# facebookresearch/foundpose

Measured on AMD Instinct MI355X. Metric: detections/sec (ViT+kNN match) on 518^2 crops vs 10k-template bank, higher is better.
Workload: dtype bf16; 1 GPU; tie_order=torch

## Files before the change

### foundpose_amd/_lib.py

```python

import ctypes as C
import os

import torch

_HERE = os.path.dirname(os.path.abspath(__file__))
LIB_PATH = os.environ.get("FOUNDPOSE_AMD_LIB") or os.path.join(_HERE, "lib", "libfoundpose_amd.so")

FP_F32, FP_BF16, FP_FP8, FP_F16X3, FP_F16F8, FP_F16 = 0, 1, 2, 3, 4, 5
GEMM_SPLIT_F16F8 = 1 << 20
GEMM_F16 = 1 << 21
SPLIT_SCALE_ACT, SPLIT_SCALE_QKV, SPLIT_SCALE_HID = 16.0, 16.0, 4.0
ABI_VERSION = 20

vp, i32, i64, f32, f64, u64 = C.c_void_p, C.c_int, C.c_int64, C.c_float, C.c_double, C.c_uint64


class VitBlock(C.Structure):
    _fields_ = [(n, vp) for n in (
        "ln1_w", "ln1_b", "ln2_w", "ln2_b", "ls1", "ls2",
        "qkv_w", "proj_w", "fc1_w", "fc2_w",
        "qkv_b", "proj_b", "fc1_b", "fc2_b", "qkv_s", "proj_s", "fc1_s", "fc2_s")] + [("act_scale", f32 * 4), ("qkv_colsum", vp), ("fc1_colsum", vp)]


# ... 23 lines not shown
    "fp_cosine_topk_prefiltered": [vp, vp, vp, i32, i32, vp, vp, vp, i32, i32, i32, i32, vp, vp, vp, i32, vp],
    "fp_cyclic_buddies": [vp, vp, vp, vp, i32, i32, vp, vp, vp, i32, vp, vp, vp, vp, i32, i32, i32, i32,
                          vp, vp, vp, vp, vp, vp, vp, vp, i32, vp],
    "fp_pack_records": [vp, vp, vp, vp, vp, vp, vp, vp, vp, i32, i32, i32, vp, vp],
    "fp_pnp_ransac": [vp, vp, vp, vp, i32, i32, i32, i32, f64, f64, i32, i32, u64, vp, vp, vp, vp, vp, vp, vp],
    "fp_pnp_ransac_keyed": [vp, vp, vp, vp, vp, i32, i32, i32, i32, f64, f64, i32, i32, u64, vp, vp, vp, vp, vp, vp, vp],
    "fp_kabsch_ransac": [vp, vp, vp, vp, vp, vp, vp, vp, vp, i32, i32, i32, vp, i32, i32, i32, i32, f64, i32, i32, u64, vp, vp, vp, vp, vp, vp, vp, vp],
    "fp_pose_verify_depth": [vp, vp, vp, vp, vp, vp, vp, vp, vp, vp, vp, i32, vp, i32, i32, i32, i32, i32, i32, i32, vp, vp, vp, vp],
    "fp_pose_verify_mask": [vp, vp, vp, vp, vp, vp, vp, vp, vp, i32, vp, vp, i32, i32, i32, i32, i32, i32, vp, vp, vp, vp],
    "fp_sample_bilinear": [vp, i64, i64, i64, i64, i32, i32, i32, i32, i32, vp, vp, i32, vp, vp],
    "fp_pca_project": [vp, i32, i32, vp, i32, vp, vp, vp],
    "fp_vit_forward": [C.POINTER(VitModel), C.POINTER(VitWorkspace), vp, i32, i32, i32, i32, vp],
    "fp_vit_sample_features": [C.POINTER(VitModel), C.POINTER(VitWorkspace), i32, i32, i32, i32, i32, i32, vp, vp, i32, vp, vp],
    "fp_query_select": [vp, i32, i32, i32, vp, vp, vp, i32, vp, i32, i32, vp, vp, vp, vp, vp, vp, vp, vp, vp],
    "fp_vit_forward_prefix": [C.POINTER(VitModel), C.POINTER(VitWorkspace), vp, i32, i32, i32, i32, vp],
    "fp_vit_block_selected": [C.POINTER(VitModel), C.POINTER(VitWorkspace), i32, i32, i32, i32, vp, vp, i32, i32, vp],
    "fp_vit_sample_features_selected": [C.POINTER(VitModel), C.POINTER(VitWorkspace), i32, i32, i32, i32, i32, i32, vp, vp, i32, vp, vp, vp],
    "fp_vit_features": [C.POINTER(VitModel), C.POINTER(VitWorkspace), i32, i32, i32, vp, vp, vp],
    "fp_patchify": [vp, i32, i32, i32, i32, vp, i32, i32, vp],
    "fp_layernorm": [vp, i32, vp, vp, f32, vp, i32, i32, i32, i32, i32, i32, i32, vp],
    "fp_gemm_bf16": [vp, i32, vp, i32, i32, i32, i32, i32, vp, vp, vp, i32, i32, vp],
    "fp_gemm_bf16_ln": [vp, i32, vp, i32, i32, i32, i32, i32, vp, vp, i32, i32, vp, vp, vp, i32, vp, vp],
    "fp_gemm_resid_tile_rows": [i32, i32, i32],
    "fp_ln_finalize": [vp, i32, i32, i32, i32, f32, vp, vp],
    "fp_gemm_fp8": [vp, i32, vp, i32, i32, i32, i32, i32, vp, vp, vp, i32, i32, f32, vp],
    "fp_quantize_fp8": [vp, i32, i64, f32, vp, vp],
    "fp_gemm_split": [vp, i32, vp, i32, i32, i32, i32, i32, vp, vp, vp, i32, i32, f32, f32, vp],
    "fp_attention_split": [vp, i32, vp, i32, i32, i32, i32, i32, f32, f32, i32, vp],
    "fp_layernorm_scaled": [vp, i32, vp, vp, f32, vp, i32, i32, f32, i32, i32, vp],
    "fp_gemm_f32": [vp, i32, vp, i32, i32, i32, i32, vp, vp, vp, i32, i32, vp],
    "fp_attention": [vp, i32, vp, i32, i32, i32, i32, i32, i32, vp],
    "fp_convert_f32_to_bf16": [vp, vp, i64, vp],
    "fp_warp_crops": [vp, i32, i32, i32, i32, i32, vp, vp, i32, i32, i32, i32, vp, vp, vp],
    "fp_warp_depth": [vp, i32, i32, vp, vp, i32, i32, i32, i32, vp, vp],
    "fp_render_setup": [vp, vp, vp, i32, vp, i32, vp, i32, i32, i32, vp, vp, vp, vp, vp, vp, vp, vp, vp, vp, vp, vp],
    "fp_render_raster": [vp, vp, vp, i32, vp, i32, vp, i32, i32, i32, vp, vp, vp, vp, vp, vp, vp, vp, vp, vp, vp, vp],
    "fp_texture_mips": [vp, i32, i32, vp, vp],
    "fp_render_raster_textured": [vp, vp, vp, i32, vp, i32, vp, i32, i32, i32, vp, vp, vp, vp, vp, vp, vp, vp, vp, vp, vp, vp, vp,
                                  i32, i32, vp, vp],
    "fp_template_downsample": [vp, vp, vp, i32, i32, i32, i32, vp, vp, vp, vp, vp],
    "fp_pose_errors": [vp, i32, vp, vp, vp, vp, i32, vp, i32, vp, C.c_size_t, vp, vp, vp],
    "fp_vsd_counts": [vp, i32, vp, i32, vp, i32, i32, i32, vp, vp, i32, vp, i32, vp, C.c_size_t, vp, vp],
    "fp_featuremetric_refine": [vp, i64, i64, i64, i64, i32, i32, i32, i32, i32, vp, vp, vp, vp, vp, vp, vp, i64, vp, i32, i32, i32,
                                vp, C.c_size_t, vp, vp, vp, vp, vp, vp, vp, vp, vp],
    "fp_depth_refine": [vp, i32, i32, i32, vp, vp, vp, vp, vp, vp, vp, i64, vp, vp, i32, i32, i32, vp, C.c_size_t, vp, vp, vp, vp, vp, vp, vp, vp, vp],
    "fp_rgbd_refine": [vp, i64, i64, i64, i64, i32, i32, i32, i32, i32, vp, vp, vp, vp, i32, i32, i32, vp, vp, vp, vp, vp, vp, vp, vp, i64, vp, vp, C.c_double,
# ... 143 lines not shown
```

### foundpose_amd/csrc/api.cpp

```cpp
#include <cmath>
#include <cstdarg>
#include <cstdio>
#include <cstring>
#include <cstdlib>
#include <vector>

#include "../../include/foundpose_amd.h"
#include "common.hpp"
#include "kernels.hpp"

static thread_local char g_err[512] = "";

void fp_set_error(const char* fmt, ...) {
  va_list ap;
  va_start(ap, fmt);
  vsnprintf(g_err, sizeof(g_err), fmt, ap);
  va_end(ap);
}

#define ST(s) reinterpret_cast<hipStream_t>(s)
#define TRY(expr)              \
  do {                         \
    int rc__ = (expr);         \
    if (rc__ != FP_OK) return rc__; \
// ... 288 lines not shown
  return patchify_launch(images, B, H, W, patch, out, ld_out, out_dtype, ST(stream), (out_dtype == FP_DTYPE_F16X3 || out_dtype == FP_DTYPE_F16F8) ? FP_SPLIT_SCALE_ACT : 1.f);
}

int fp_layernorm(const float* x, int ld_x, const float* weight, const float* bias, float eps, void* out, int ld_out,
                 int out_dtype, int dim, int out_rows, int out_rows_per_img, int in_rows_per_img, int in_skip,
                 fp_stream_t stream) {
  FP_REQUIRE(x && weight && bias && out, "fp_layernorm: null pointer");
  LayerNormArgs a;
  memset(&a, 0, sizeof(a));
  a.x = x; a.ld_x = ld_x; a.weight = weight; a.bias = bias; a.eps = eps; a.out = out; a.ld_out = ld_out;
  a.out_dtype = out_dtype; a.out_scale = 0.f; a.dim = dim; a.out_rows = out_rows;
  a.out_rows_per_img = out_rows_per_img > 0 ? out_rows_per_img : (out_rows > 0 ? out_rows : 1);
  a.in_rows_per_img = in_rows_per_img > 0 ? in_rows_per_img : a.out_rows_per_img;
  a.in_skip = in_skip;
  return layernorm_launch(a, ST(stream));
}

int fp_gemm_bf16(const void* A, int lda, const void* W, int ldw, int M, int N, int K, int M_valid, const float* bias,
                 const float* gamma, void* out, int ldo, int epilogue, fp_stream_t stream) {
  FP_REQUIRE(A && W && out, "fp_gemm_bf16: null pointer");
  const int tile = (epilogue >> 8) & 0xfff;
  const bool f16 = (epilogue >> 21) & 1;
  epilogue &= 0xff;
  FP_REQUIRE(tile == 0 || tile == 64 || tile == 128 || tile == 256 || tile == 320, "fp_gemm_bf16: bad tile override %d", tile);

  FP_REQUIRE(epilogue == GEMM_EPI_BIAS_BF16 || epilogue == GEMM_EPI_GELU_BF16 || epilogue == GEMM_EPI_LS_RESID_F32 ||
                 epilogue == GEMM_EPI_BIAS_F32 || epilogue == GEMM_EPI_SWIGLU_BF16,
             "fp_gemm_bf16: epilogue %d is not available through this entry point", epilogue);
  FP_REQUIRE(epilogue != GEMM_EPI_LS_RESID_F32 || gamma, "fp_gemm_bf16: gamma required");
  GemmBf16Args a;
  memset(&a, 0, sizeof(a));
  a.A = reinterpret_cast<const __bf16*>(A); a.lda = lda; a.W = reinterpret_cast<const __bf16*>(W); a.ldw = ldw;
  a.M = M; a.N = N; a.K = K; a.M_valid = M_valid; a.bias = bias; a.gamma = gamma; a.out = out; a.ldo = ldo;
  a.tile_override = tile;
  return gemm_launch(f16 ? GemmFmt::F16 : GemmFmt::BF16, epilogue, a, ST(stream));
}

int fp_gemm_bf16_ln(const void* A, int lda, const void* W, int ldw, int M, int N, int K, int M_valid, const float* bias, void* out, int ldo,
                    int epilogue, const float* colsum, const float* ln_row, void* xb, int ld_xb, float* stats, fp_stream_t stream) {
  FP_REQUIRE(A && W && out && bias, "fp_gemm_bf16_ln: null pointer");
  const int tile = (epilogue >> 8) & 0xfff;
  const bool f16 = (epilogue >> 21) & 1;
  epilogue &= 0xff;
  FP_REQUIRE(tile == 0 || tile == 64 || tile == 128 || tile == 256 || tile == 320 || (tile == 352 && epilogue == GEMM_EPI_RESID_HILO), "fp_gemm_bf16_ln: bad tile override %d", tile);
  GemmBf16Args a;
  memset(&a, 0, sizeof(a));
  a.A = reinterpret_cast<const __bf16*>(A); a.lda = lda; a.W = reinterpret_cast<const __bf16*>(W); a.ldw = ldw;
  a.M = M; a.N = N; a.K = K; a.M_valid = M_valid; a.bias = bias; a.out = out; a.ldo = ldo; a.tile_override = tile;
  if (epilogue == GEMM_EPI_RESID_HILO) {
    FP_REQUIRE(xb && stats, "fp_gemm_bf16_ln: epilogue 8 needs xb, out (= the low halves) and stats");
    a.xb = reinterpret_cast<__bf16*>(xb); a.ld_xb = ld_xb; a.xl = reinterpret_cast<__bf16*>(out); a.stats_out = reinterpret_cast<float2*>(stats);
    a.out = nullptr;
  } else if (epilogue == GEMM_EPI_RESID_F32) {
    FP_REQUIRE((xb == nullptr) == (stats == nullptr), "fp_gemm_bf16_ln: xb and stats go together");
    FP_REQUIRE(!xb || (N % 128 == 0 && ld_xb >= N && ld_xb % 4 == 0), "fp_gemm_bf16_ln: N must be a multiple of 128 and ld_xb cover the row");
    a.xb = reinterpret_cast<__bf16*>(xb); a.ld_xb = ld_xb; a.stats_out = reinterpret_cast<float2*>(stats);
  } else {
    FP_REQUIRE(epilogue == GEMM_EPI_BIAS_BF16 || epilogue == GEMM_EPI_GELU_BF16 || epilogue == GEMM_EPI_SWIGLU_BF16,
               "fp_gemm_bf16_ln: epilogue %d has no folded-LayerNorm form", epilogue);
    FP_REQUIRE(colsum && ln_row, "fp_gemm_bf16_ln: colsum and ln_row are required");
    a.colsum = colsum; a.ln_stats = reinterpret_cast<const float2*>(ln_row); a.ln_eps = 1e-6f;
  }
  return gemm_launch(f16 ? GemmFmt::F16 : GemmFmt::BF16, epilogue, a, ST(stream));
}

int fp_gemm_resid_tile_rows(int M_valid, int N, int num_cus) { return gemm_resid_tile_rows(M_valid, N, num_cus); }

int fp_ln_finalize(const float* stats, int parts, int stats_stride, int rows, int dim, float eps, float* ln_row, fp_stream_t stream) {
  FP_REQUIRE(stats && ln_row && parts >= 1 && dim >= 1, "fp_ln_finalize: bad arguments");
  return ln_finalize_launch(reinterpret_cast<const float2*>(stats), parts, stats_stride, rows, dim, eps, reinterpret_cast<float2*>(ln_row), ST(stream));
}

#ifdef FP_GEMM_TIMELINE
int fp_gemm_bf16_timeline(const void* A, int lda, const void* W, int ldw, int M, int N, int K, int M_valid, const float* bias,
                          const float* gamma, void* out, int ldo, int epilogue, unsigned long long* dbg, int64_t dbg_len,
                          fp_stream_t stream) {
  FP_REQUIRE(A && W && out && dbg, "fp_gemm_bf16_timeline: null pointer");
  FP_REQUIRE(dbg_len >= 4ll * ((M + 127) / 128) * ((N + 127) / 128) * 2, "fp_gemm_bf16_timeline: stamp buffer too small");
  GemmBf16Args a;
  memset(&a, 0, sizeof(a));
  a.A = reinterpret_cast<const __bf16*>(A); a.lda = lda; a.W = reinterpret_cast<const __bf16*>(W); a.ldw = ldw;
  a.M = M; a.N = N; a.K = K; a.M_valid = M_valid; a.bias = bias; a.gamma = gamma; a.out = out; a.ldo = ldo;
  a.tile_override = (epilogue >> 8) & 0xfff;
  a.dbg = dbg;
  return gemm_launch(GemmFmt::BF16, epilogue & 0xff, a, ST(stream));
}
#endif

int fp_gemm_fp8(const void* A, int lda, const void* W, int ldw, int M, int N, int K, int M_valid, const float* bias,
// ... 722 lines not shown
```

### foundpose_amd/csrc/gemm_bf16.hip

```cpp
#include "gemm_kernel.hpp"

int gemm_resid_tile_rows(int m_valid, int n, int cus) { return resid_tile_rows(m_valid, n, cus); }

template int gemm_launch_fmt<GemmFmt::BF16>(int epi, const GemmBf16Args& a, hipStream_t st);
```

### foundpose_amd/csrc/gemm_kernel.hpp

```cpp
#pragma once
#include "common.hpp"
#include "kernels.hpp"
#include <type_traits>

namespace {

constexpr int BK = 64;

typedef __attribute__((address_space(3))) void lds_void;

FP_DEVICE int swz(int row) { return (row >> 1) & 7; }

FP_DEVICE unsigned stage_lane_offset(int ld, int lane, int parity) {
  const int row_l = lane >> 3;
  const int chunk = (lane & 7) ^ ((4 * parity + (row_l >> 1)) & 7);
  return (unsigned)(row_l * ld + chunk * 8) * 2u;
}
FP_DEVICE void stage_rows(__amdgpu_buffer_rsrc_t rsrc, unsigned voff, int ld, int row0, int k0, char* lds, int rblk) {
  const unsigned soff = (unsigned)((row0 + rblk * 8) * ld + k0) * 2u;
  __builtin_amdgcn_raw_ptr_buffer_load_lds(rsrc, (lds_void*)(lds + rblk * 1024), 16, voff, soff, 0, 0);
}

FP_DEVICE bf16x8 read_frag(const char* lds, int row, int chunk) {
  return *reinterpret_cast<const bf16x8*>(lds + row * 128 + ((chunk ^ swz(row)) << 4));
}

FP_DEVICE f32x2 gelu_pk(f32x2 x) {
  constexpr float X = 3.9f;
  f32x2 xc;
  xc[0] = __builtin_amdgcn_fmed3f(x[0], -X, X);
  xc[1] = __builtin_amdgcn_fmed3f(x[1], -X, X);
  const f32x2 s = xc * xc;
  f32x2 q = f32x2{3.214934915e-08f, 3.214934915e-08f};
  q = __builtin_elementwise_fma(q, s, f32x2{-2.075321994e-06f, -2.075321994e-06f});
  q = __builtin_elementwise_fma(q, s, f32x2{5.740229389e-05f, 5.740229389e-05f});
  q = __builtin_elementwise_fma(q, s, f32x2{-9.056365499e-04f, -9.056365499e-04f});
  q = __builtin_elementwise_fma(q, s, f32x2{9.218766509e-03f, 9.218766509e-03f});
  q = __builtin_elementwise_fma(q, s, f32x2{-6.556460516e-02f, -6.556460516e-02f});
  q = __builtin_elementwise_fma(q, s, f32x2{3.986083959e-01f, 3.986083959e-01f});
  const f32x2 phi = __builtin_elementwise_fma(xc, q, f32x2{0.5f, 0.5f});
  return x * phi;
}
// ... 54 lines not shown
  return v;
}

typedef __attribute__((ext_vector_type(8))) int i32x8;
typedef __attribute__((ext_vector_type(4))) int i32x4;

template <int EPI, int BM, int BN, int WM, int WN, GemmFmt FMT, bool F8OUT = false, int NSTAGE = 2>
__global__ __launch_bounds__(WM * WN * 64, 2) void gemm_bf16_kernel(GemmBf16Args a) {
  constexpr bool F8 = FMT == GemmFmt::FP8, SX = FMT == GemmFmt::F16F8, SP = FMT == GemmFmt::F16X3 || SX, H16 = FMT == GemmFmt::F16;
  constexpr bool SPOUT = SP && (EPI == GEMM_EPI_BIAS_BF16 || EPI == GEMM_EPI_GELU_BF16 || EPI == GEMM_EPI_SWIGLU_BF16);
  static_assert(NSTAGE == 2 || (NSTAGE == 4 && !F8 && !SP && WM * WN != 8), "the deep pipeline exists for the small bf16 / fp16 tiles");
  static_assert(!F8OUT || (F8 && (EPI == GEMM_EPI_GELU_BF16 || EPI == GEMM_EPI_SWIGLU_BF16)), "fp8 output: GELU / SwiGLU epilogues of the fp8 kernels");
  constexpr int NW = WM * WN, NT = NW * 64, MT = BM / 32, TM = (MT + WM - 1) / WM, WROWS = TM * 32, TN = BN / WN / 32;
  constexpr bool UNEVEN = MT % WM != 0;
  static_assert(BM % 32 == 0 && (!UNEVEN || (WM == 2 && FMT != GemmFmt::FP8 && FMT != GemmFmt::F16X3 && FMT != GemmFmt::F16F8)), "uneven wave rows: the bf16 / fp16 loop of the 2 x 4 wave grid");
  constexpr bool HILO = EPI == GEMM_EPI_RESID_HILO;
  constexpr bool RESID = EPI == GEMM_EPI_LS_RESID_F32 || EPI == GEMM_EPI_RESID_F32 || HILO;
  constexpr int A_BYTES = BM * BK * 2, B_BYTES = BN * BK * 2, STAGE = A_BYTES + B_BYTES;
  constexpr bool ASYM = NW == 8;
  constexpr int NISSUE = ASYM ? NW / 2 : NW;
  constexpr int A_INSTR = BM / 8 / NISSUE, B_INSTR = BN / 8 / NISSUE;
  constexpr int PIECES = A_INSTR + B_INSTR;
  static_assert(PIECES % 2 == 0 || !(F8 || SP), "staging split");
  extern __shared__ __attribute__((aligned(16))) char smem[];
  const int tid = threadIdx.x, lane = tid & 63, wave = __builtin_amdgcn_readfirstlane(tid >> 6);
  const int wm = wave / WN, wn = wave % WN, l31 = lane & 31, kh = lane >> 5;
  auto tile_on = [&](int i) { return !UNEVEN || wm * TM + i < MT; };

  const unsigned nwg = gridDim.x;
  const unsigned lid = xcd_remap(blockIdx.x, nwg);
  const unsigned tiles_n = a.N / BN;
  int m0, n0;
  if (a.rast_r) {
    const unsigned per = a.rast_r * a.rast_gn, st = lid / per, r = lid - st * per;
    const unsigned SM = (a.m_tiles + a.rast_r - 1) / a.rast_r;
    const unsigned sn = st / SM, sm = st - sn * SM;
    const unsigned tm = sm * a.rast_r + r % a.rast_r, tn = sn * a.rast_gn + r / a.rast_r;
    if (tm >= (unsigned)a.m_tiles) return;
    m0 = tm * BM;
    n0 = tn * BN;
  } else {
    m0 = (lid / tiles_n) * BM;
    n0 = (lid % tiles_n) * BN;
  }
  const int kb = 0, ke = a.K / BK;

// ... 2 lines not shown
  if (a.dbg) ts0 = __builtin_readcyclecounter();
#endif
  {
    f32x16 acc[TM][TN];
#pragma unroll
    for (int i = 0; i < TM; ++i)
#pragma unroll
      for (int j = 0; j < TN; ++j)
#pragma unroll
        for (int r = 0; r < 16; ++r) acc[i][j][r] = 0.f;

    constexpr bool A_ILV = A_INSTR % 2 != 0;
    static_assert((A_INSTR % 2 == 0 || (NISSUE % 2 == 0 && BM / 8 % NISSUE == 0)) && B_INSTR % 2 == 0, "row-group parity of a piece must be a compile-time (or per-wave) property");
    auto tile_rsrc = [](const __bf16* base, int row0, int rows, int ld) {
      const unsigned long long bytes = (unsigned long long)(rows - row0) * ld * 2ull;
      return __builtin_amdgcn_make_buffer_rsrc((void*)(base + (size_t)row0 * ld), 0, bytes > 0xffffffffull ? 0xffffffffu : (unsigned)bytes, 0x00020000);
    };
    const __amdgpu_buffer_rsrc_t rsrc_a = tile_rsrc(a.A, m0, a.M, a.lda), rsrc_w = tile_rsrc(a.W, n0, a.N, a.ldw);
    const unsigned voff_a[2] = {stage_lane_offset(a.lda, lane, 0), stage_lane_offset(a.lda, lane, 1)};
    const unsigned voff_w[2] = {stage_lane_offset(a.ldw, lane, 0), stage_lane_offset(a.ldw, lane, 1)};
    const bool issuer = !ASYM || wm == 0;
    const int iw = ASYM ? wave % NISSUE : wave;
    const unsigned voff_a_w = voff_a[iw & 1];
    auto stage_piece = [&](int q, int t, char* buf) {
      if (!issuer) return;
      if (q < A_INSTR) {
        if constexpr (A_ILV) stage_rows(rsrc_a, voff_a_w, a.lda, 0, t * BK, buf, q * NISSUE + iw);
        else stage_rows(rsrc_a, voff_a[q & 1], a.lda, 0, t * BK, buf, iw * A_INSTR + q);
      }
      else stage_rows(rsrc_w, voff_w[(q - A_INSTR) & 1], a.ldw, 0, t * BK, buf + A_BYTES, iw * B_INSTR + (q - A_INSTR));
    };
#pragma unroll
    for (int q = 0; q < PIECES; ++q) stage_piece(q, kb, smem);
    if constexpr (NSTAGE > 2) {
#pragma unroll
      for (int d = 1; d < NSTAGE - 1; ++d)
        if (kb + d < ke) {
#pragma unroll
          for (int q = 0; q < PIECES; ++q) stage_piece(q, kb + d, smem + d * STAGE);
        }
    }

    float ln_rs[TM], ln_mrs[TM];
#pragma unroll
    for (int i = 0; i < TM; ++i) { ln_rs[i] = 1.f; ln_mrs[i] = 0.f; }
    if constexpr (!F8 && (EPI == GEMM_EPI_BIAS_BF16 || EPI == GEMM_EPI_GELU_BF16 || EPI == GEMM_EPI_SWIGLU_BF16)) {
      if (a.ln_stats) {
#pragma unroll
        for (int i = 0; i < TM; ++i) {
          if (!tile_on(i)) continue;
          const float2 st = a.ln_stats[m0 + wm * WROWS + i * 32 + l31];
          ln_rs[i] = st.x;
          ln_mrs[i] = st.y;
          if constexpr (H16) {
            ln_rs[i] *= a.acc_scale;
            ln_mrs[i] *= a.acc_scale;
          }
        }
      }
    }

    if constexpr (UNEVEN) {
      static_assert(NSTAGE == 2 && !F8 && !SP, "uneven wave rows: the two-stage bf16 / fp16 loop");
      auto k_loop = [&](auto tmw) {
        constexpr int TMW = decltype(tmw)::value;
        for (int t = kb; t < ke; ++t) {
          const int cur = (t - kb) & 1;
          asm volatile("s_waitcnt vmcnt(0)" ::: "memory");
          __syncthreads();
          char* nxt = smem + (cur ^ 1) * STAGE;
          const bool more = t + 1 < ke;
          const char* As = smem + cur * STAGE;
          const char* Ws = As + A_BYTES;
#pragma unroll
// ... 171 lines not shown
        }
      }
        }
      __syncthreads();
    }
#ifdef FP_GEMM_TIMELINE
    if (a.dbg) ts2 = __builtin_readcyclecounter();
#endif

    constexpr bool USE_SLAB = EPI == GEMM_EPI_BIAS_BF16 || EPI == GEMM_EPI_GELU_BF16 ||
                              EPI == GEMM_EPI_SWIGLU_BF16 || RESID;
    static_assert(!F8 || USE_SLAB, "the fp8 kernels exist for the slab epilogues only");
    if constexpr (USE_SLAB) {
    constexpr bool OUT_F32 = RESID || EPI == GEMM_EPI_TOKENS_F32 || EPI == GEMM_EPI_BIAS_F32;
    constexpr int ESZ = OUT_F32 ? 4 : (F8OUT ? 1 : (SPOUT ? 4 : 2));
    constexpr int OUT_COLS = EPI == GEMM_EPI_SWIGLU_BF16 ? BN / 2 : BN;
    constexpr int SLAB_ROWS = WM * 32, SLAB_STRIDE = OUT_COLS * ESZ + 16;
    constexpr int CHUNKS_PER_ROW = OUT_COLS * ESZ / 16, SLAB_CHUNKS = SLAB_ROWS * CHUNKS_PER_ROW, NT = NW * 64;
    static_assert(SLAB_ROWS * SLAB_STRIDE <= 2 * STAGE, "slab must fit the main-loop LDS");
    constexpr bool TWO_SLABS = 2 * SLAB_ROWS * SLAB_STRIDE <= 2 * STAGE;
    constexpr int SLAB_BYTES = SLAB_ROWS * SLAB_STRIDE;
    constexpr bool LN_FOLD_OK = !F8 && (EPI == GEMM_EPI_BIAS_BF16 || EPI == GEMM_EPI_GELU_BF16 || EPI == GEMM_EPI_SWIGLU_BF16);
    const bool fold = LN_FOLD_OK && a.ln_stats != nullptr;
    constexpr bool BIAS_LATE = TM * TN * 16 > 160;
    float4 bias[TN][4], gam[TN][4];
  #pragma unroll
    for (int tn = 0; tn < TN; ++tn)
  #pragma unroll
      for (int g = 0; g < 4; ++g) {
        const int n = n0 + wn * (BN / WN) + tn * 32 + 8 * g + 4 * kh;
        if constexpr (!BIAS_LATE) bias[tn][g] = *reinterpret_cast<const float4*>(a.bias + n);
        if constexpr (EPI == GEMM_EPI_LS_RESID_F32 || F8) gam[tn][g] = *reinterpret_cast<const float4*>(a.gamma + n);
        if constexpr (LN_FOLD_OK) {
          if (fold) gam[tn][g] = *reinterpret_cast<const float4*>(a.colsum + n);
        }
      }
    __syncthreads();
    float sat_amax = 0.f;
  #pragma unroll
    for (int tm = 0; tm < TM; ++tm) {
      const int m = m0 + wm * WROWS + tm * 32 + l31;
      float band_amax = 0.f;
      constexpr int PASSES = (SLAB_CHUNKS + NT - 1) / NT;
      static_assert(SLAB_CHUNKS % NT == 0, "slab chunks must divide evenly over the block");
      float4 ext[PASSES];
      int orow_i[PASSES];
      constexpr int CPR8 = HILO ? OUT_COLS / 8 : 1, PASS8 = HILO ? SLAB_ROWS * CPR8 / NT : 1;
      uint4 exh[PASS8], exl[PASS8];
      if constexpr (HILO) {
        static_assert(!HILO || (SLAB_ROWS * CPR8) % NT == 0, "slab chunks must divide evenly over the block");
  #pragma unroll
        for (int it = 0; it < PASS8; ++it) {
          const int id = tid + it * NT;
          const int r = id / CPR8, c = id - r * CPR8;
          const int gm_row = m0 + (r >> 5) * WROWS + tm * 32 + (r & 31);
          const bool okr = gm_row < a.M_valid && (!UNEVEN || (r >> 5) * TM + tm < MT);
// ... 10 lines not shown
        const int r = id / CHUNKS_PER_ROW, c = id - r * CHUNKS_PER_ROW;
        const int gm_row = m0 + (r >> 5) * WROWS + tm * 32 + (r & 31);
        const bool okr = gm_row < a.M_valid && (!UNEVEN || (r >> 5) * TM + tm < MT);
        int orow = gm_row;
        if constexpr (EPI == GEMM_EPI_TOKENS_F32) {
          const int b = gm_row / a.tok_np, pidx = gm_row - b * a.tok_np;
          orow = b * a.tok_n + a.tok_skip + pidx;
          if (okr) ext[it] = *reinterpret_cast<const float4*>(a.pos + (size_t)pidx * a.ldo + n0 + c * 4);
        }
        if constexpr (RESID) {
          if (okr) ext[it] = *reinterpret_cast<const float4*>(reinterpret_cast<const float*>(a.out) + (size_t)orow * a.ldo + n0 + c * 4);
        }
        orow_i[it] = okr ? orow : -1;
      }
      const float rs = ln_rs[tm], mrs = ln_mrs[tm];
      char* slab = smem + (TWO_SLABS ? (tm & 1) * SLAB_BYTES : 0);
      char* srow = slab + (wm * 32 + l31) * SLAB_STRIDE;
  #pragma unroll
      for (int tn = 0; tn < TN; ++tn)
  #pragma unroll
        for (int g = 0; g < 4; ++g) {
          const int col = wn * (BN / WN) + tn * 32 + 8 * g + 4 * kh;
          float4 bs;
          if constexpr (BIAS_LATE) bs = *reinterpret_cast<const float4*>(a.bias + n0 + col);
          else bs = bias[tn][g];
          float v0 = acc[tm][tn][4 * g + 0] + bs.x, v1 = acc[tm][tn][4 * g + 1] + bs.y;
          float v2 = acc[tm][tn][4 * g + 2] + bs.z, v3 = acc[tm][tn][4 * g + 3] + bs.w;
          if constexpr (SP || H16) {
            const float as = a.acc_scale;
            v0 = fmaf(acc[tm][tn][4 * g + 0], as, bs.x); v1 = fmaf(acc[tm][tn][4 * g + 1], as, bs.y);
            v2 = fmaf(acc[tm][tn][4 * g + 2], as, bs.z); v3 = fmaf(acc[tm][tn][4 * g + 3], as, bs.w);
          }
          if constexpr (LN_FOLD_OK) {
            if (fold) {
              const float4 cs = gam[tn][g];
              const f32x2 rs2 = {rs, rs}, nm2 = {-mrs, -mrs};
              const f32x2 t01 = __builtin_elementwise_fma(nm2, f32x2{cs.x, cs.y}, f32x2{bs.x, bs.y});
              const f32x2 t23 = __builtin_elementwise_fma(nm2, f32x2{cs.z, cs.w}, f32x2{bs.z, bs.w});
              const f32x2 r01 = __builtin_elementwise_fma(rs2, f32x2{acc[tm][tn][4 * g + 0], acc[tm][tn][4 * g + 1]}, t01);
              const f32x2 r23 = __builtin_elementwise_fma(rs2, f32x2{acc[tm][tn][4 * g + 2], acc[tm][tn][4 * g + 3]}, t23);
              v0 = r01[0]; v1 = r01[1]; v2 = r23[0]; v3 = r23[1];
            }
          }
          if constexpr (F8 && EPI != GEMM_EPI_LS_RESID_F32) {
            const float4 gm = gam[tn][g];
            v0 *= gm.x; v1 *= gm.y; v2 *= gm.z; v3 *= gm.w;
          }
          if constexpr (EPI == GEMM_EPI_GELU_BF16) {
            if constexpr (H16) {
              const f32x2 g01 = gelu_pk9(f32x2{v0, v1}), g23 = gelu_pk9(f32x2{v2, v3});
              v0 = g01[0]; v1 = g01[1]; v2 = g23[0]; v3 = g23[1];
            } else if constexpr (SP) {
              const f32x2 g01 = gelu_erf_pk(f32x2{v0, v1}), g23 = gelu_erf_pk(f32x2{v2, v3});
              v0 = g01[0]; v1 = g01[1]; v2 = g23[0]; v3 = g23[1];
            } else {
              const f32x2 g01 = gelu_pk(f32x2{v0, v1}), g23 = gelu_pk(f32x2{v2, v3});
              v0 = g01[0]; v1 = g01[1]; v2 = g23[0]; v3 = g23[1];
            }
// ... 178 lines not shown
struct GemmRaster { int r, gn; };
static GemmRaster pick_raster(int bm, int n_tiles, unsigned grid) {
  const int wide8 = n_tiles % 8 == 0;
  const int rr = wide8 ? 4 : 8, gn = wide8 ? 8 : 4;
  if (bm >= 256 && n_tiles % gn == 0 && n_tiles > 4 && grid >= 512) return {rr, gn};
  return {0, 0};
}

template <int EPI, int BM, int BN, int WM, int WN, GemmFmt FMT, bool F8OUT = false, int NSTAGE = 2>
int launch_cfg(const GemmBf16Args& a_in, hipStream_t st) {
  GemmBf16Args a = a_in;
  if constexpr (FMT == GemmFmt::F16) {
    if (!(a.acc_scale > 0.f)) a.acc_scale = 1.f;
  }
  a.m_tiles = (a.M + BM - 1) / BM;
  if (a.M_valid > 0 && (a.M_valid + BM - 1) / BM < a.m_tiles) a.m_tiles = (a.M_valid + BM - 1) / BM;
  unsigned grid = a.m_tiles * (a.N / BN);
  a.rast_r = a.rast_gn = 0;
  const GemmRaster ra = pick_raster(BM, a.N / BN, grid);
  if (ra.r) {
    a.rast_r = ra.r; a.rast_gn = ra.gn;
    grid = ((a.m_tiles + ra.r - 1) / ra.r) * ((a.N / BN) / ra.gn) * 32;
  }
  const size_t lds = (size_t)(BM + BN) * BK * 2 * NSTAGE;
  static FpDeviceOnce attr;
  fp_allow_dynamic_lds(attr, &gemm_bf16_kernel<EPI, BM, BN, WM, WN, FMT, F8OUT, NSTAGE>, (int)lds);
  hipLaunchKernelGGL((gemm_bf16_kernel<EPI, BM, BN, WM, WN, FMT, F8OUT, NSTAGE>), dim3(grid), dim3(WM * WN * 64), lds, st, a);
  FP_CHECK_LAUNCH("gemm_bf16_kernel");
  return FP_OK;
}

static int xcd_rounds(int bm, int m_valid, int n_tiles, int cus) {
  const int m_tiles = (m_valid + bm - 1) / bm, xcds = 8, per_xcd = cus / xcds > 0 ? cus / xcds : 32;
  const GemmRaster ra = pick_raster(bm, n_tiles, (unsigned)(m_tiles * n_tiles));
  if (ra.r) return (((m_tiles + ra.r - 1) / ra.r) * (n_tiles / ra.gn) + xcds - 1) / xcds;
  const int chunk = (m_tiles * n_tiles + xcds - 1) / xcds;
  return (chunk + per_xcd - 1) / per_xcd;
}
static bool tall_tile_wins(const GemmBf16Args& a) {
  if (a.M % 320 != 0 || a.M % 256 != 0 || a.N % 256 != 0) return false;
  const int cus = fp_num_cus();
  return (float)(xcd_rounds(320, a.M_valid, a.N / 256, cus) * 320) * 0.97f < (float)(xcd_rounds(256, a.M_valid, a.N / 256, cus) * 256);
}

static int resid_tile_rows(int m_valid, int n, int cus) {
  if (m_valid <= 0 || n <= 0 || n % 256 != 0 || cus <= 0) return 256;
  const int r352 = xcd_rounds(352, m_valid, n / 256, cus), r256 = xcd_rounds(256, m_valid, n / 256, cus);
  return r352 < r256 && r352 * 352 < r256 * 256 ? 352 : 256;
}

template <int EPI, GemmFmt FMT>
int launch(const GemmBf16Args& a, hipStream_t st) {
  constexpr bool SP = FMT == GemmFmt::F16X3 || FMT == GemmFmt::F16F8;
  const int force = a.tile_override;
  const bool big_ok = a.M % 256 == 0 && a.N % 256 == 0;
  const int tiles_big = (a.M / 256) * (a.N / 256), cus = fp_num_cus();
  const bool use_big = big_ok && (force == 256 || (force == 0 && tiles_big >= cus && !(tiles_big > cus && tiles_big < cus + cus / 2)));
  if constexpr (!SP && (EPI == GEMM_EPI_BIAS_BF16 || EPI == GEMM_EPI_GELU_BF16 || EPI == GEMM_EPI_RESID_HILO)) {
    if ((force == 320 && a.M % 320 == 0 && a.N % 256 == 0) || (force == 0 && use_big && tall_tile_wins(a)))
      return launch_cfg<EPI, 320, 256, 2, 4, FMT>(a, st);
  }
  if constexpr (!SP && EPI == GEMM_EPI_RESID_HILO) {
    const bool ok352 = a.N % 256 == 0 && a.M_valid > 0 && a.M_valid <= a.M;
    if (ok352 && (force == 352 || (force == 0 && use_big && resid_tile_rows(a.M_valid, a.N, cus) == 352)))
      return launch_cfg<EPI, 352, 256, 2, 4, FMT>(a, st);
    FP_REQUIRE(force != 352, "gemm_bf16: the 352-row tile needs N %% 256 == 0 and 0 < M_valid <= M (N %d, M_valid %d, M %d)", a.N, a.M_valid, a.M);
  }
  if (use_big) return launch_cfg<EPI, 256, 256, 2, 4, FMT>(a, st);
  if constexpr (!SP && (EPI == GEMM_EPI_RESID_HILO || EPI == GEMM_EPI_RESID_F32 || EPI == GEMM_EPI_LS_RESID_F32)) {
    const int tiles_128 = (a.M_valid > 0 ? (a.M_valid + 127) / 128 : a.M / 128) * (a.N / 128);
    if ((force == 64 && a.M % 64 == 0) || (force == 0 && a.M % 64 == 0 && tiles_128 <= cus / 2))
      return launch_cfg<EPI, 64, 128, 2, 2, FMT, false, 4>(a, st);
  }
  return launch_cfg<EPI, 128, 128, 2, 2, FMT>(a, st);
}

template <int EPI, bool F8OUT = false>
int launch_fp8(const GemmBf16Args& a, hipStream_t st) {
  if constexpr (EPI != GEMM_EPI_LS_RESID_F32) {
    if (a.tile_override == 320 ? a.M % 320 == 0 : (a.tile_override == 0 && tall_tile_wins(a)))
      return launch_cfg<EPI, 320, 256, 2, 4, GemmFmt::FP8, F8OUT>(a, st);
// ... 75 lines not shown
```

### foundpose_amd/csrc/kernels.hpp

```cpp
#pragma once
#include <hip/hip_runtime.h>
#include <stdint.h>

#include "../../include/foundpose_amd.h"

enum : int {
  F32_EPI_STORE = 0,
  F32_EPI_DIST_STORE = 1,
  F32_EPI_DIST_ARGMIN = 2,
  F32_EPI_SUB_VEC = 3,
  F32_EPI_BIAS = 4,
  F32_EPI_BIAS_GELU = 5,
  F32_EPI_LS_RESID = 6,
  F32_EPI_TOKENS = 7,
  F32_EPI_SWIGLU = 8,
  F32_EPI_DIST_TOPK = 9,
};

struct F32TileArgs {
  const float* A; int lda;
  const float* B; int ldb;
  int K, M, N;
  const int* a_seg_off; const int* pair_a_seg; int pair_a_div;
  const int* b_seg_off; const int* pair_b_seg;
// ... 112 lines not shown
  int tile_override;
  int m_tiles;
  unsigned rast_r, rast_gn;
  float out_scale;
  float acc_scale;
  unsigned long long* dbg;
  __bf16* xb; int ld_xb;
  __bf16* xl;
  float2* stats_out;
  const float2* ln_stats; int ln_parts; float ln_eps;
  const float* colsum;
  int* sat;
};

enum class GemmFmt {
  BF16,
  F16,
  FP8,
  F16X3,
  F16F8,
};
template <GemmFmt FMT> int gemm_launch_fmt(int epi, const GemmBf16Args& a, hipStream_t st);
int gemm_resid_tile_rows(int m_valid, int n, int cus);
int gemm_launch(GemmFmt fmt, int epi, const GemmBf16Args& a, hipStream_t st);

enum : int { FP_DTYPE_F32 = 0, FP_DTYPE_BF16 = 1, FP_DTYPE_FP8 = 2, FP_DTYPE_F16X3 = 3, FP_DTYPE_F16F8 = 4,
             FP_DTYPE_F16 = 5 };

struct AttnArgs {
  const void* qkv; int ld_qkv;
  void* out; int ld_out;
  int batch, n_tok, dim, heads;
  float out_fp8_scale;
  const int* sel_rows; const int* sel_off; int max_sel;
  int variant;
  int tail_last;
  float in_scale, out_scale;
  int out_fmt;
  int* sat;
};
int attn_launch(const AttnArgs& a, int dtype, hipStream_t st);

struct LayerNormArgs {
  const float* x; int ld_x;
  const float* weight; const float* bias; float eps;
  void* out; int ld_out; int out_dtype;
// ... 230 lines not shown
```

### foundpose_amd/ops.py

```python

from typing import Optional, Tuple

import torch

from . import _lib
from ._lib import call, knn_scratch_bytes, ptr, stream, require_cuda


def _f32c(t: torch.Tensor) -> torch.Tensor:
    if t.dtype != torch.float32:
        t = t.float()
    return t if t.is_contiguous() else t.contiguous()


def sqnorm_rows(x: torch.Tensor) -> torch.Tensor:
    require_cuda(x)
    x = _f32c(x)
    out = torch.empty(x.shape[0], dtype=torch.float32, device=x.device)
    call("fp_sqnorm_rows", ptr(x), x.shape[0], x.shape[1], ptr(out), stream())
    return out


def normalize_rows(x: torch.Tensor, eps: float = 1e-8) -> torch.Tensor:
    require_cuda(x)
# ... 74 lines not shown
    call("fp_pca_project", ptr(x), x.shape[0], x.shape[1], ptr(components), components.shape[0], ptr(mean_proj),
         ptr(out), stream())
    return out


def gemm_f32(a: torch.Tensor, w: torch.Tensor, bias=None, gamma=None, out=None, epilogue: int = 0) -> torch.Tensor:
    require_cuda(a, w)
    M, K = a.shape
    N = w.shape[0]
    if out is None:
        out = torch.empty(M, N, dtype=torch.float32, device=a.device)
    call("fp_gemm_f32", ptr(a), a.stride(0), ptr(w), w.stride(0), M, N, K, ptr(bias), ptr(gamma), ptr(out),
         out.stride(0), epilogue, stream())
    return out


def _h16_bit(a: torch.Tensor, w: torch.Tensor) -> int:
    if a.dtype != w.dtype or a.dtype not in (torch.bfloat16, torch.float16):
        raise ValueError("the 16-bit GEMMs take two bf16 or two fp16 operands")
    return _lib.GEMM_F16 if a.dtype == torch.float16 else 0


def gemm_bf16(a: torch.Tensor, w: torch.Tensor, bias: torch.Tensor, gamma=None, out=None, epilogue: int = 0,
              m_valid: Optional[int] = None) -> torch.Tensor:
    require_cuda(a, w, bias)
    M, K = a.shape
    N = w.shape[0]
    if out is None:
        dt = torch.float32 if (epilogue & 0xff) in (3, 5) else a.dtype
        out = torch.zeros(M, N // 2 if (epilogue & 0xff) == 6 else N, dtype=dt, device=a.device)
    call("fp_gemm_bf16", ptr(a), a.stride(0), ptr(w), w.stride(0), M, N, K, M if m_valid is None else m_valid,
         ptr(bias), ptr(gamma), ptr(out), out.stride(0), epilogue | _h16_bit(a, w), stream())
    return out


def gemm_bf16_resid_ln(a: torch.Tensor, w: torch.Tensor, bias: torch.Tensor, x: torch.Tensor, emit: bool = True, tile: int = 0, m_valid: Optional[int] = None):
    require_cuda(a, w, bias, x)
    M, K = a.shape
    N = w.shape[0]
    xb = torch.zeros(M, N, dtype=a.dtype, device=a.device) if emit else None
    stats = torch.zeros(N // 128, M, 2, dtype=torch.float32, device=a.device) if emit else None
    call("fp_gemm_bf16_ln", ptr(a), a.stride(0), ptr(w), w.stride(0), M, N, K, M if m_valid is None else m_valid, ptr(bias), ptr(x), x.stride(0),
         7 | (tile << 8) | _h16_bit(a, w), None, None, ptr(xb), N, ptr(stats), stream())
    return xb, stats


def gemm_bf16_resid_hilo(a: torch.Tensor, w: torch.Tensor, bias: torch.Tensor, xb: torch.Tensor, xl: torch.Tensor, tile: int = 0, m_valid: Optional[int] = None):
    require_cuda(a, w, bias, xb, xl)
    M, K = a.shape
    N = w.shape[0]
    if xb.dtype != a.dtype or xl.dtype != a.dtype or xb.stride(0) != xl.stride(0):
        raise ValueError("xb / xl are arrays of the operands' 16-bit type with one row stride")
    if xb.stride(0) % 8 or xb.data_ptr() % 16 or xl.data_ptr() % 16 or xb.stride(1) != 1 or xl.stride(1) != 1:
        raise ValueError("xb / xl: 16-byte aligned rows (row stride a multiple of 8 elements, unit column stride) -- the epilogue moves 8 bf16 per access")
    stats = torch.zeros(N // 128, M, 2, dtype=torch.float32, device=a.device)
# ... 221 lines not shown
```

### include/foundpose_amd.h

```cpp
#ifndef FOUNDPOSE_AMD_H
#define FOUNDPOSE_AMD_H

#include <stddef.h>
#include <stdint.h>

#ifdef __cplusplus
extern "C" {
#endif

typedef void* fp_stream_t;

enum { FP_F32 = 0, FP_BF16 = 1, FP_FP8 = 2, FP_F16X3 = 3, FP_F16F8 = 4, FP_F16 = 5 };

#define FP_SPLIT_SCALE_ACT 16.f
#define FP_SPLIT_SCALE_QKV 16.f
#define FP_SPLIT_SCALE_HID 4.f

#define FP_GEMM_SPLIT_F16F8 (1 << 20)

#define FP_GEMM_F16 (1 << 21)

#define FP_ABI_VERSION 20
int fp_abi_version(void);
const char* fp_last_error(void);
// ... 129 lines not shown
                           int img_h, const float* points, const int32_t* point_img, int num_points, float* out, fp_stream_t stream);

int fp_query_select(const uint8_t* masks, int B, int H, int W, const int32_t* pix_x, const int32_t* pix_y, const float* grid_points, int num_points,
                    const int64_t* point_cells, int num_cells, int n_tok, int32_t* scratch, int32_t* counts, float* out_points, int32_t* out_point_img,
                    int32_t* out_q_off, int32_t* sel_rows, int32_t* sel_off, int32_t* row_map, fp_stream_t stream);
int fp_vit_forward_prefix(const fp_vit_model* model, const fp_vit_workspace* ws, const float* images, int B, int H, int W, int layer,
                          fp_stream_t stream);
int fp_vit_block_selected(const fp_vit_model* model, const fp_vit_workspace* ws, int B, int H, int W, int layer, const int32_t* sel_rows,
                          const int32_t* sel_off, int num_sel, int max_sel_per_img, fp_stream_t stream);
int fp_vit_sample_features_selected(const fp_vit_model* model, const fp_vit_workspace* ws, int B, int grid_h, int grid_w, int apply_norm,
                                    int img_w, int img_h, const float* points, const int32_t* point_img, int num_points,
                                    const int32_t* row_map, float* out, fp_stream_t stream);

int fp_patchify(const float* images, int B, int H, int W, int patch, void* out, int ld_out, int out_dtype,
                fp_stream_t stream);
int fp_layernorm(const float* x, int ld_x, const float* weight, const float* bias, float eps, void* out, int ld_out,
                 int out_dtype, int dim, int out_rows, int out_rows_per_img, int in_rows_per_img, int in_skip,
                 fp_stream_t stream);
int fp_gemm_bf16(const void* A, int lda, const void* W, int ldw, int M, int N, int K, int M_valid, const float* bias,
                 const float* gamma, void* out, int ldo, int epilogue, fp_stream_t stream);
int fp_gemm_bf16_ln(const void* A, int lda, const void* W, int ldw, int M, int N, int K, int M_valid, const float* bias, void* out, int ldo,
                    int epilogue, const float* colsum, const float* ln_row, void* xb, int ld_xb, float* stats, fp_stream_t stream);
int fp_gemm_resid_tile_rows(int M_valid, int N, int num_cus);
int fp_ln_finalize(const float* stats, int parts, int stats_stride, int rows, int dim, float eps, float* ln_row, fp_stream_t stream);

int fp_gemm_fp8(const void* A, int lda, const void* W, int ldw, int M, int N, int K, int M_valid, const float* bias,
                const float* col_scale, void* out, int ldo, int epilogue, float out_scale, fp_stream_t stream);
int fp_gemm_split(const void* A, int lda, const void* W, int ldw, int M, int N, int K, int M_valid, const float* bias, const float* gamma,
                  void* out, int ldo, int epilogue, float acc_scale, float out_scale, fp_stream_t stream);
int fp_attention_split(const void* qkv, int ld_qkv, void* out, int ld_out, int B, int n_tok, int dim, int heads, float in_scale, float out_scale,
                       int out_dtype, fp_stream_t stream);
int fp_layernorm_scaled(const float* x, int ld_x, const float* weight, const float* bias, float eps, void* out, int ld_out, int out_dtype, float out_scale,
                        int dim, int out_rows, fp_stream_t stream);
int fp_quantize_fp8(const void* in, int in_dtype, int64_t n, float scale, void* out, fp_stream_t stream);
int fp_gemm_f32(const float* A, int lda, const float* W, int ldw, int M, int N, int K, const float* bias,
                const float* gamma, float* out, int ldo, int epilogue, fp_stream_t stream);
#define FP_ATTN_VARIANT(v) ((v) << 8)
int fp_attention(const void* qkv, int ld_qkv, void* out, int ld_out, int B, int n_tok,
                 int dim, int heads, int dtype, fp_stream_t stream);
int fp_convert_f32_to_bf16(const float* in, void* out, int64_t n, fp_stream_t stream);

enum { FP_WARP_LINEAR = 0, FP_WARP_NEAREST = 1 };
int fp_warp_crops(const void* src, int n_src, int src_h, int src_w, int channels, int mode, const int32_t* src_index,
                  const double* params, int batch, int out_h, int out_w, int depth_check, void* out, float* map_out,
                  fp_stream_t stream);

// ... 101 lines not shown
```

Measured before the change: 1157 detections/s.

## Add 352/320-row tile selection for bias and GELU GEMMs with LDS-stashed bias

Extends the tall 352-row and 320-row GEMM tile configurations, previously used only for the residual epilogue, to the bias and GELU epilogues such as QKV and FC1. A cost heuristic weighs XCD-round counts and per-raster correction factors to choose among 256, 320 and 352 rows. For wide tiles, the bias and LN colsum vectors are stashed in LDS rather than held in registers, and A-row staging is clamped to valid rows so tiles past M stay in bounds. The goal is to cut wave quantization and tail rounds across CUs, at the cost of more LDS use and heuristic tuning constants that may not fit every shape.

```diff
diff --git a/foundpose_amd/_lib.py b/foundpose_amd/_lib.py
--- a/foundpose_amd/_lib.py
+++ b/foundpose_amd/_lib.py
@@ -69,6 +69,7 @@
     "fp_gemm_bf16": [vp, i32, vp, i32, i32, i32, i32, i32, vp, vp, vp, i32, i32, vp],
     "fp_gemm_bf16_ln": [vp, i32, vp, i32, i32, i32, i32, i32, vp, vp, i32, i32, vp, vp, vp, i32, vp, vp],
     "fp_gemm_resid_tile_rows": [i32, i32, i32],
+    "fp_gemm_wide_tile_rows": [i32, i32, i32, i32],
     "fp_ln_finalize": [vp, i32, i32, i32, i32, f32, vp, vp],
     "fp_gemm_fp8": [vp, i32, vp, i32, i32, i32, i32, i32, vp, vp, vp, i32, i32, f32, vp],
     "fp_quantize_fp8": [vp, i32, i64, f32, vp, vp],
diff --git a/foundpose_amd/csrc/api.cpp b/foundpose_amd/csrc/api.cpp
--- a/foundpose_amd/csrc/api.cpp
+++ b/foundpose_amd/csrc/api.cpp
@@ -334,7 +334,8 @@
   const int tile = (epilogue >> 8) & 0xfff;
   const bool f16 = (epilogue >> 21) & 1;
   epilogue &= 0xff;
-  FP_REQUIRE(tile == 0 || tile == 64 || tile == 128 || tile == 256 || tile == 320, "fp_gemm_bf16: bad tile override %d", tile);
+  FP_REQUIRE(tile == 0 || tile == 64 || tile == 128 || tile == 256 || tile == 320 || (tile == 352 && (epilogue == GEMM_EPI_BIAS_BF16 || epilogue == GEMM_EPI_GELU_BF16)),
+             "fp_gemm_bf16: bad tile override %d", tile);
 
   FP_REQUIRE(epilogue == GEMM_EPI_BIAS_BF16 || epilogue == GEMM_EPI_GELU_BF16 || epilogue == GEMM_EPI_LS_RESID_F32 ||
                  epilogue == GEMM_EPI_BIAS_F32 || epilogue == GEMM_EPI_SWIGLU_BF16,
@@ -354,7 +355,9 @@
   const int tile = (epilogue >> 8) & 0xfff;
   const bool f16 = (epilogue >> 21) & 1;
   epilogue &= 0xff;
-  FP_REQUIRE(tile == 0 || tile == 64 || tile == 128 || tile == 256 || tile == 320 || (tile == 352 && epilogue == GEMM_EPI_RESID_HILO), "fp_gemm_bf16_ln: bad tile override %d", tile);
+  FP_REQUIRE(tile == 0 || tile == 64 || tile == 128 || tile == 256 || tile == 320 ||
+                 (tile == 352 && (epilogue == GEMM_EPI_RESID_HILO || epilogue == GEMM_EPI_BIAS_BF16 || epilogue == GEMM_EPI_GELU_BF16)),
+             "fp_gemm_bf16_ln: bad tile override %d", tile);
   GemmBf16Args a;
   memset(&a, 0, sizeof(a));
   a.A = reinterpret_cast<const __bf16*>(A); a.lda = lda; a.W = reinterpret_cast<const __bf16*>(W); a.ldw = ldw;
@@ -377,6 +380,7 @@
 }
 
 int fp_gemm_resid_tile_rows(int M_valid, int N, int num_cus) { return gemm_resid_tile_rows(M_valid, N, num_cus); }
+int fp_gemm_wide_tile_rows(int M, int M_valid, int N, int num_cus) { return gemm_wide_tile_rows(M, M_valid, N, num_cus); }
 
 int fp_ln_finalize(const float* stats, int parts, int stats_stride, int rows, int dim, float eps, float* ln_row, fp_stream_t stream) {
   FP_REQUIRE(stats && ln_row && parts >= 1 && dim >= 1, "fp_ln_finalize: bad arguments");
diff --git a/foundpose_amd/csrc/gemm_bf16.hip b/foundpose_amd/csrc/gemm_bf16.hip
--- a/foundpose_amd/csrc/gemm_bf16.hip
+++ b/foundpose_amd/csrc/gemm_bf16.hip
@@ -1,5 +1,6 @@
 #include "gemm_kernel.hpp"
 
 int gemm_resid_tile_rows(int m_valid, int n, int cus) { return resid_tile_rows(m_valid, n, cus); }
+int gemm_wide_tile_rows(int m, int m_valid, int n, int cus) { return wide_tile_rows(m, m_valid, n, cus); }
 
 template int gemm_launch_fmt<GemmFmt::BF16>(int epi, const GemmBf16Args& a, hipStream_t st);
diff --git a/foundpose_amd/csrc/gemm_kernel.hpp b/foundpose_amd/csrc/gemm_kernel.hpp
--- a/foundpose_amd/csrc/gemm_kernel.hpp
+++ b/foundpose_amd/csrc/gemm_kernel.hpp
@@ -18,6 +18,10 @@
 }
 FP_DEVICE void stage_rows(__amdgpu_buffer_rsrc_t rsrc, unsigned voff, int ld, int row0, int k0, char* lds, int rblk) {
   const unsigned soff = (unsigned)((row0 + rblk * 8) * ld + k0) * 2u;
+  __builtin_amdgcn_raw_ptr_buffer_load_lds(rsrc, (lds_void*)(lds + rblk * 1024), 16, voff, soff, 0, 0);
+}
+FP_DEVICE void stage_rows_from(__amdgpu_buffer_rsrc_t rsrc, unsigned voff, int ld, int src_row, int k0, char* lds, int rblk) {
+  const unsigned soff = (unsigned)(src_row * ld + k0) * 2u;
   __builtin_amdgcn_raw_ptr_buffer_load_lds(rsrc, (lds_void*)(lds + rblk * 1024), 16, voff, soff, 0, 0);
 }
 
@@ -118,6 +122,8 @@
   constexpr int A_INSTR = BM / 8 / NISSUE, B_INSTR = BN / 8 / NISSUE;
   constexpr int PIECES = A_INSTR + B_INSTR;
   static_assert(PIECES % 2 == 0 || !(F8 || SP), "staging split");
+  constexpr bool BIAS_LDS = TM * TN * 16 > 160;
+  static_assert(!BIAS_LDS || (!F8 && !SP && NT == 2 * BN && NSTAGE == 2), "one thread per stashed value, behind two stages");
   extern __shared__ __attribute__((aligned(16))) char smem[];
   const int tid = threadIdx.x, lane = tid & 63, wave = __builtin_amdgcn_readfirstlane(tid >> 6);
   const int wm = wave / WN, wn = wave % WN, l31 = lane & 31, kh = lane >> 5;
@@ -166,10 +172,14 @@
     const bool issuer = !ASYM || wm == 0;
     const int iw = ASYM ? wave % NISSUE : wave;
     const unsigned voff_a_w = voff_a[iw & 1];
+    const int a_last_grp = (a.M - m0 < BM ? a.M - m0 : BM) - 8;
     auto stage_piece = [&](int q, int t, char* buf) {
       if (!issuer) return;
       if (q < A_INSTR) {
-        if constexpr (A_ILV) stage_rows(rsrc_a, voff_a_w, a.lda, 0, t * BK, buf, q * NISSUE + iw);
+        if constexpr (A_ILV) {
+          const int rblk = q * NISSUE + iw;
+          stage_rows_from(rsrc_a, voff_a_w, a.lda, rblk * 8 < a_last_grp ? rblk * 8 : a_last_grp, t * BK, buf, rblk);
+        }
         else stage_rows(rsrc_a, voff_a[q & 1], a.lda, 0, t * BK, buf, iw * A_INSTR + q);
       }
       else stage_rows(rsrc_w, voff_w[(q - A_INSTR) & 1], a.ldw, 0, t * BK, buf + A_BYTES, iw * B_INSTR + (q - A_INSTR));
@@ -185,6 +195,11 @@
         }
     }
 
+    if constexpr (BIAS_LDS) {
+      float* stash = reinterpret_cast<float*>(smem + 2 * STAGE);
+      if (tid < BN) stash[tid] = a.bias[n0 + tid];
+      else if (a.colsum) stash[tid] = a.colsum[n0 + tid - BN];
+    }
     float ln_rs[TM], ln_mrs[TM];
 #pragma unroll
     for (int i = 0; i < TM; ++i) { ln_rs[i] = 1.f; ln_mrs[i] = 0.f; }
@@ -193,7 +208,11 @@
 #pragma unroll
         for (int i = 0; i < TM; ++i) {
           if (!tile_on(i)) continue;
-          const float2 st = a.ln_stats[m0 + wm * WROWS + i * 32 + l31];
+          const int row = m0 + wm * WROWS + i * 32 + l31;
+          if constexpr (UNEVEN) {
+            if (row >= a.M_valid) continue;
+          }
+          const float2 st = a.ln_stats[row];
           ln_rs[i] = st.x;
           ln_mrs[i] = st.y;
           if constexpr (H16) {
@@ -411,16 +430,15 @@
     constexpr int SLAB_BYTES = SLAB_ROWS * SLAB_STRIDE;
     constexpr bool LN_FOLD_OK = !F8 && (EPI == GEMM_EPI_BIAS_BF16 || EPI == GEMM_EPI_GELU_BF16 || EPI == GEMM_EPI_SWIGLU_BF16);
     const bool fold = LN_FOLD_OK && a.ln_stats != nullptr;
-    constexpr bool BIAS_LATE = TM * TN * 16 > 160;
     float4 bias[TN][4], gam[TN][4];
   #pragma unroll
     for (int tn = 0; tn < TN; ++tn)
   #pragma unroll
       for (int g = 0; g < 4; ++g) {
         const int n = n0 + wn * (BN / WN) + tn * 32 + 8 * g + 4 * kh;
-        if constexpr (!BIAS_LATE) bias[tn][g] = *reinterpret_cast<const float4*>(a.bias + n);
+        if constexpr (!BIAS_LDS) bias[tn][g] = *reinterpret_cast<const float4*>(a.bias + n);
         if constexpr (EPI == GEMM_EPI_LS_RESID_F32 || F8) gam[tn][g] = *reinterpret_cast<const float4*>(a.gamma + n);
-        if constexpr (LN_FOLD_OK) {
+        if constexpr (LN_FOLD_OK && !BIAS_LDS) {
           if (fold) gam[tn][g] = *reinterpret_cast<const float4*>(a.colsum + n);
         }
       }
@@ -477,7 +495,7 @@
         for (int g = 0; g < 4; ++g) {
           const int col = wn * (BN / WN) + tn * 32 + 8 * g + 4 * kh;
           float4 bs;
-          if constexpr (BIAS_LATE) bs = *reinterpret_cast<const float4*>(a.bias + n0 + col);
+          if constexpr (BIAS_LDS) bs = *reinterpret_cast<const float4*>(smem + 2 * STAGE + col * 4);
           else bs = bias[tn][g];
           float v0 = acc[tm][tn][4 * g + 0] + bs.x, v1 = acc[tm][tn][4 * g + 1] + bs.y;
           float v2 = acc[tm][tn][4 * g + 2] + bs.z, v3 = acc[tm][tn][4 * g + 3] + bs.w;
@@ -488,7 +506,9 @@
           }
           if constexpr (LN_FOLD_OK) {
             if (fold) {
-              const float4 cs = gam[tn][g];
+              float4 cs;
+              if constexpr (BIAS_LDS) cs = *reinterpret_cast<const float4*>(smem + 2 * STAGE + (BN + col) * 4);
+              else cs = gam[tn][g];
               const f32x2 rs2 = {rs, rs}, nm2 = {-mrs, -mrs};
               const f32x2 t01 = __builtin_elementwise_fma(nm2, f32x2{cs.x, cs.y}, f32x2{bs.x, bs.y});
               const f32x2 t23 = __builtin_elementwise_fma(nm2, f32x2{cs.z, cs.w}, f32x2{bs.z, bs.w});
@@ -713,7 +733,8 @@
     a.rast_r = ra.r; a.rast_gn = ra.gn;
     grid = ((a.m_tiles + ra.r - 1) / ra.r) * ((a.N / BN) / ra.gn) * 32;
   }
-  const size_t lds = (size_t)(BM + BN) * BK * 2 * NSTAGE;
+  constexpr bool BIAS_LDS = (BM / 32 + WM - 1) / WM * (BN / WN / 32) * 16 > 160;
+  const size_t lds = (size_t)(BM + BN) * BK * 2 * NSTAGE + (BIAS_LDS ? 2 * BN * 4 : 0);
   static FpDeviceOnce attr;
   fp_allow_dynamic_lds(attr, &gemm_bf16_kernel<EPI, BM, BN, WM, WN, FMT, F8OUT, NSTAGE>, (int)lds);
   hipLaunchKernelGGL((gemm_bf16_kernel<EPI, BM, BN, WM, WN, FMT, F8OUT, NSTAGE>), dim3(grid), dim3(WM * WN * 64), lds, st, a);
@@ -738,6 +759,23 @@
   if (m_valid <= 0 || n <= 0 || n % 256 != 0 || cus <= 0) return 256;
   const int r352 = xcd_rounds(352, m_valid, n / 256, cus), r256 = xcd_rounds(256, m_valid, n / 256, cus);
   return r352 < r256 && r352 * 352 < r256 * 256 ? 352 : 256;
+}
+
+constexpr float WIDE_FACTOR_320 = 0.97f, WIDE_FACTOR_352_R8X4 = 1.02f, WIDE_FACTOR_352_R4X8 = 1.05f;
+static int wide_tile_rows(int m, int m_valid, int n, int cus) {
+  if (m <= 0 || m % 256 != 0 || m_valid <= 0 || m_valid > m || n <= 0 || n % 256 != 0 || cus <= 0) return 256;
+  const int tiles_big = (m / 256) * (n / 256);
+  if (tiles_big < cus || (tiles_big > cus && tiles_big < cus + cus / 2)) return 256;
+  int best = 256;
+  float cost = (float)(xcd_rounds(256, m_valid, n / 256, cus) * 256);
+  if (m % 320 == 0) {
+    const float c320 = (float)(xcd_rounds(320, m_valid, n / 256, cus) * 320) * WIDE_FACTOR_320;
+    if (c320 < cost) { best = 320; cost = c320; }
+  }
+  const GemmRaster ra = pick_raster(352, n / 256, (unsigned)((m_valid + 351) / 352 * (n / 256)));
+  const float c352 = (float)(xcd_rounds(352, m_valid, n / 256, cus) * 352) * (ra.gn == 8 ? WIDE_FACTOR_352_R4X8 : WIDE_FACTOR_352_R8X4);
+  if (ra.r && c352 < cost) best = 352;
+  return best;
 }
 
 template <int EPI, GemmFmt FMT>
@@ -747,7 +785,14 @@
   const bool big_ok = a.M % 256 == 0 && a.N % 256 == 0;
   const int tiles_big = (a.M / 256) * (a.N / 256), cus = fp_num_cus();
   const bool use_big = big_ok && (force == 256 || (force == 0 && tiles_big >= cus && !(tiles_big > cus && tiles_big < cus + cus / 2)));
-  if constexpr (!SP && (EPI == GEMM_EPI_BIAS_BF16 || EPI == GEMM_EPI_GELU_BF16 || EPI == GEMM_EPI_RESID_HILO)) {
+  if constexpr (!SP && (EPI == GEMM_EPI_BIAS_BF16 || EPI == GEMM_EPI_GELU_BF16)) {
+    const int pick = force == 0 && use_big ? wide_tile_rows(a.M, a.M_valid, a.N, cus) : 0;
+    const bool ok352 = a.N % 256 == 0 && a.M_valid > 0 && a.M_valid <= a.M;
+    if (ok352 && (force == 352 || pick == 352)) return launch_cfg<EPI, 352, 256, 2, 4, FMT>(a, st);
+    FP_REQUIRE(force != 352, "gemm_bf16: the 352-row tile needs N %% 256 == 0 and 0 < M_valid <= M (N %d, M_valid %d, M %d)", a.N, a.M_valid, a.M);
+    if ((force == 320 && a.M % 320 == 0 && a.N % 256 == 0) || pick == 320) return launch_cfg<EPI, 320, 256, 2, 4, FMT>(a, st);
+  }
+  if constexpr (!SP && EPI == GEMM_EPI_RESID_HILO) {
     if ((force == 320 && a.M % 320 == 0 && a.N % 256 == 0) || (force == 0 && use_big && tall_tile_wins(a)))
       return launch_cfg<EPI, 320, 256, 2, 4, FMT>(a, st);
   }
diff --git a/foundpose_amd/csrc/kernels.hpp b/foundpose_amd/csrc/kernels.hpp
--- a/foundpose_amd/csrc/kernels.hpp
+++ b/foundpose_amd/csrc/kernels.hpp
@@ -158,6 +158,7 @@
 };
 template <GemmFmt FMT> int gemm_launch_fmt(int epi, const GemmBf16Args& a, hipStream_t st);
 int gemm_resid_tile_rows(int m_valid, int n, int cus);
+int gemm_wide_tile_rows(int m, int m_valid, int n, int cus);
 int gemm_launch(GemmFmt fmt, int epi, const GemmBf16Args& a, hipStream_t st);
 
 enum : int { FP_DTYPE_F32 = 0, FP_DTYPE_BF16 = 1, FP_DTYPE_FP8 = 2, FP_DTYPE_F16X3 = 3, FP_DTYPE_F16F8 = 4,
diff --git a/foundpose_amd/ops.py b/foundpose_amd/ops.py
--- a/foundpose_amd/ops.py
+++ b/foundpose_amd/ops.py
@@ -120,7 +120,7 @@
 
 
 def gemm_bf16(a: torch.Tensor, w: torch.Tensor, bias: torch.Tensor, gamma=None, out=None, epilogue: int = 0,
-              m_valid: Optional[int] = None) -> torch.Tensor:
+              m_valid: Optional[int] = None, tile: int = 0) -> torch.Tensor:
     require_cuda(a, w, bias)
     M, K = a.shape
     N = w.shape[0]
@@ -128,7 +128,7 @@
         dt = torch.float32 if (epilogue & 0xff) in (3, 5) else a.dtype
         out = torch.zeros(M, N // 2 if (epilogue & 0xff) == 6 else N, dtype=dt, device=a.device)
     call("fp_gemm_bf16", ptr(a), a.stride(0), ptr(w), w.stride(0), M, N, K, M if m_valid is None else m_valid,
-         ptr(bias), ptr(gamma), ptr(out), out.stride(0), epilogue | _h16_bit(a, w), stream())
+         ptr(bias), ptr(gamma), ptr(out), out.stride(0), epilogue | (tile << 8) | _h16_bit(a, w), stream())
     return out
 
 
diff --git a/include/foundpose_amd.h b/include/foundpose_amd.h
--- a/include/foundpose_amd.h
+++ b/include/foundpose_amd.h
@@ -175,6 +175,7 @@
 int fp_gemm_bf16_ln(const void* A, int lda, const void* W, int ldw, int M, int N, int K, int M_valid, const float* bias, void* out, int ldo,
                     int epilogue, const float* colsum, const float* ln_row, void* xb, int ld_xb, float* stats, fp_stream_t stream);
 int fp_gemm_resid_tile_rows(int M_valid, int N, int num_cus);
+int fp_gemm_wide_tile_rows(int M, int M_valid, int N, int num_cus);
 int fp_ln_finalize(const float* stats, int parts, int stats_stride, int rows, int dim, float eps, float* ln_row, fp_stream_t stream);
 
 int fp_gemm_fp8(const void* A, int lda, const void* W, int ldw, int M, int N, int K, int M_valid, const float* bias,
```

New measurement: 1169 detections/s (median of 6 runs). +1.0%, better.
